# arobertlin/MinPaxos

Measured on AMD Instinct MI355X. Metric: decided+applied instances/sec (tally + KV apply + RCCL watermark all-reduce), higher is better.
Workload: dtype int32/int64

## Files before the change

minpaxos_amd/csrc/logenc.hip:

```cpp
#include <cstring>

#include "common.hpp"
#include "frames.hpp"
#include "kernels.hpp"
#include "scan.hpp"

namespace mpx {

namespace {
constexpr int kLogBlock = kFrBlock;
constexpr int kLogWindowVec = 2;
constexpr int kLogBlockBytes = kLogBlock * 16 * kLogWindowVec;
constexpr int kLogMinRec = 9;
constexpr int kLogMaxRecs = kLogBlockBytes / kLogMinRec + 2;
constexpr int kLogMaxCmds = kLogBlockBytes / 17 + 3;

__host__ __device__ __forceinline__ uint64_t zigzag(int64_t x) {
    return x < 0 ? ~((uint64_t)x << 1) : (uint64_t)x << 1;
}
__host__ __device__ __forceinline__ uint32_t hdr_bytes(int format, uint64_t ncmd) {
    return format == MPX_LOG_CATCHUP ? 8u + uvarint_len(zigzag((int64_t)ncmd)) : 12u;
}
}

struct RecBytes {
    int format;
    const uint64_t* cmd_off;
    __device__ __forceinline__ uint64_t operator()(uint64_t i) const {
        const uint64_t nc = cmd_off[i + 1] - cmd_off[i];
        return hdr_bytes(format, nc) + 17 * nc;
    }
};
struct RecOffOut {
    uint64_t* rec_off;
    uint64_t* blk_first;
    uint32_t n_blocks;
    __device__ __forceinline__ void operator()(uint64_t i, uint64_t s, uint64_t bytes) const {
        const uint64_t e = s + bytes;
        rec_off[i + 1] = e;
        for (uint64_t b = (s + kLogBlockBytes - 1) / kLogBlockBytes;
             b * kLogBlockBytes < e && b < n_blocks; ++b)
            blk_first[b] = i;
    }
};

__global__ __launch_bounds__(kLogBlock) void k_log_emit(
    int format, const mpx_log_rec* __restrict__ recs, const uint64_t* __restrict__ cmd_off,
    const uint8_t* __restrict__ op, const int64_t* __restrict__ key,
    const int64_t* __restrict__ val, uint64_t n, const uint64_t* __restrict__ rec_off,
    const uint64_t* __restrict__ blk_first, uint32_t n_blocks, uint8_t* __restrict__ out) {
    __shared__ uint64_t off[kLogMaxRecs + 1];
    __shared__ uint64_t coff[kLogMaxRecs + 1];
    __shared__ uint16_t cmap[kLogMaxCmds];
    __shared__ __attribute__((aligned(16))) uint32_t W[kLogBlockBytes / 4];
    const uint64_t total = rec_off[n];
    const uint64_t b0 = (uint64_t)blockIdx.x * kLogBlockBytes;
    if (b0 >= total) return;
    const uint64_t first = blk_first[blockIdx.x];
    const uint64_t b1 = b0 + kLogBlockBytes < total ? b0 + kLogBlockBytes : total;
    const uint64_t nr = (b1 < total && blockIdx.x + 1 < n_blocks)
                            ? blk_first[blockIdx.x + 1] - first + 1
                            : n - first;
    for (uint64_t k = threadIdx.x; k <= nr; k += kLogBlock) {
        off[k] = rec_off[first + k];
        coff[k] = cmd_off[first + k];
    }
#pragma unroll
    for (int i = 0; i < kLogWindowVec; ++i)
        reinterpret_cast<uint4*>(W)[threadIdx.x + i * kLogBlock] = make_uint4(0, 0, 0, 0);
    __syncthreads();
    uint64_t j_lo, j_hi;
    {
        const uint64_t hb0 = off[1] - off[0] - 17 * (coff[1] - coff[0]);
        const uint64_t cs0 = off[0] + hb0;
        j_lo = coff[0] + cmd_span(cs0, b0, b1).lo;
        const uint64_t L = nr - 1;
        const uint64_t hbl = off[L + 1] - off[L] - 17 * (coff[L + 1] - coff[L]);
        const uint64_t csl = off[L] + hbl;
        const uint64_t c = cmd_span(csl, b0, b1).hi;
        j_hi = coff[L] + c < coff[L + 1] ? coff[L] + c : coff[L + 1];
    }
    for (uint64_t k = threadIdx.x; k < nr; k += kLogBlock) {
        const uint64_t rs = off[k], c0 = coff[k], c1 = coff[k + 1], nc = c1 - c0;
        for (uint64_t j = c0 > j_lo ? c0 : j_lo; j < c1 && j < j_hi; ++j)
            cmap[j - j_lo] = (uint16_t)k;
        const uint32_t hb = (uint32_t)(off[k + 1] - rs - 17 * nc);
        if (rs + hb <= b0 || rs >= b1) continue;
        const mpx_log_rec m = recs[first + k];
        uint32_t h[5] = {(uint32_t)m.ballot, (uint32_t)m.status, 0u, 0u, 0u};
        if (format == MPX_LOG_DURABLE) {
            h[2] = (uint32_t)m.inst_no;
        } else {
            const uint64_t zz = zigzag((int64_t)nc);
            for (uint32_t q = 0; q + 8 < hb; ++q) h[2 + (q >> 2)] |= uvarint_byte(zz, q) << (8 * (q & 3));
        }
        image_or<kLogBlockBytes / 4>(W, (int64_t)(rs - b0), h, hb);
    }
    __syncthreads();
    for (uint64_t j = j_lo + threadIdx.x; j < j_hi; j += kLogBlock) {
        const uint32_t lo = cmap[j - j_lo];
        const uint64_t nc = coff[lo + 1] - coff[lo];
        const uint64_t cs = off[lo + 1] - 17 * nc;
        const uint64_t pos = cs + 17 * (j - coff[lo]);
        image_or_cmd<kLogBlockBytes / 4>(W, (int64_t)pos - (int64_t)b0, op[j], (uint64_t)key[j],
                                         (uint64_t)val[j]);
    }
    __syncthreads();
    window_store(W, (uint32_t)(b1 - b0), out + b0, (int)threadIdx.x);
}

uint64_t logenc_max_bytes(uint64_t n, uint64_t m) { return n * (8 + 10) + 17 * m; }

namespace {
uint64_t blocks_for(uint64_t n, uint64_t m) {
    return (logenc_max_bytes(n, m) + kLogBlockBytes - 1) / kLogBlockBytes;
}
struct LogWork {
    uint64_t* blk_first;
    uint64_t* scan_tmp;
    LogWork(Carver& c, uint64_t n, uint64_t m) {
        blk_first = c.take<uint64_t>(blocks_for(n, m));
        scan_tmp = (uint64_t*)c.take<char>(scan_scratch_bytes<uint64_t>(n ? n : 1));
    }
};
}

uint64_t logenc_work_bytes(uint64_t n, uint64_t m, Carver&& c) {
    return LogWork(c, n, m), c.bytes();
}

hipError_t launch_encode_log(int format, const mpx_log_rec* recs, uint64_t n,
                             const uint64_t* cmd_off, const uint8_t* op, const int64_t* key,
                             const int64_t* val, uint64_t m, uint8_t* out, uint64_t* rec_off,
                             void* work, uint64_t work_bytes, hipStream_t stream) {
    if (format != MPX_LOG_CATCHUP && format != MPX_LOG_DURABLE) return hipErrorInvalidValue;
    Carver c(work);
    const LogWork w(c, n, m);
    if (work_bytes < c.bytes()) return hipErrorInvalidValue;
    k_zero_u64<<<1, 1, 0, stream>>>(rec_off, 1);
    if (n == 0) return hipGetLastError();
    const uint64_t blocks = blocks_for(n, m);
    const hipError_t r = device_scan(RecBytes{format, cmd_off},
                                     RecOffOut{rec_off, w.blk_first, (uint32_t)blocks}, n,
                                     ScanSum64{}, (uint64_t)0, w.scan_tmp, stream);
    if (r != hipSuccess) return r;
    k_log_emit<<<(unsigned)blocks, kLogBlock, 0, stream>>>(format, recs, cmd_off, op, key, val, n,
                                                          rec_off, w.blk_first, (uint32_t)blocks,
                                                          out);
    return hipGetLastError();
}

}
```

Before: 23.97 billion.

## Fuse log record offset scan into emit kernel with record-tiled windows

```diff
diff --git a/minpaxos_amd/csrc/logenc.hip b/minpaxos_amd/csrc/logenc.hip
--- a/minpaxos_amd/csrc/logenc.hip
+++ b/minpaxos_amd/csrc/logenc.hip
@@ -1,7 +1,10 @@
 #include <cstring>
 
 #include "common.hpp"
+#pragma clang diagnostic push
+#pragma clang diagnostic ignored "-Wunused-function"
 #include "frames.hpp"
+#pragma clang diagnostic pop
 #include "kernels.hpp"
 #include "scan.hpp"
 
@@ -13,6 +16,7 @@
 constexpr int kLogBlockBytes = kLogBlock * 16 * kLogWindowVec;
 constexpr int kLogMinRec = 9;
 constexpr int kLogMaxRecs = kLogBlockBytes / kLogMinRec + 2;
+static_assert(kLogMaxRecs <= 65536, "cmap holds 16-bit record indices");
 constexpr int kLogMaxCmds = kLogBlockBytes / 17 + 3;
 
 __host__ __device__ __forceinline__ uint64_t zigzag(int64_t x) {
@@ -23,111 +27,202 @@
 }
 }
 
-struct RecBytes {
-    int format;
-    const uint64_t* cmd_off;
-    __device__ __forceinline__ uint64_t operator()(uint64_t i) const {
-        const uint64_t nc = cmd_off[i + 1] - cmd_off[i];
-        return hdr_bytes(format, nc) + 17 * nc;
-    }
-};
-struct RecOffOut {
-    uint64_t* rec_off;
-    uint64_t* blk_first;
-    uint32_t n_blocks;
-    __device__ __forceinline__ void operator()(uint64_t i, uint64_t s, uint64_t bytes) const {
-        const uint64_t e = s + bytes;
-        rec_off[i + 1] = e;
-        for (uint64_t b = (s + kLogBlockBytes - 1) / kLogBlockBytes;
-             b * kLogBlockBytes < e && b < n_blocks; ++b)
-            blk_first[b] = i;
-    }
-};
+constexpr int kLogTile = 512;
+constexpr int kLogPer = kLogTile / kLogBlock;
+static_assert(kLogTile % kLogBlock == 0, "a whole number of records per lane");
+constexpr int kLogScanTile = 4096;
+constexpr int kLogSub = kLogScanTile / kLogTile;
+static_assert(kLogScanTile % kLogTile == 0 && kLogSub < kLogBlock, "whole emit tiles per scan tile");
+
+__device__ __forceinline__ uint64_t uniform64(uint64_t x) {
+    return (uint64_t)__builtin_amdgcn_readfirstlane((uint32_t)(x >> 32)) << 32 |
+           __builtin_amdgcn_readfirstlane((uint32_t)x);
+}
+__device__ __forceinline__ uint64_t rec_bytes(int format, uint64_t nc) {
+    return hdr_bytes(format, nc) + 17 * nc;
+}
+
+__global__ __launch_bounds__(kLogBlock) void k_log_tile_totals(
+    int format, const uint64_t* __restrict__ cmd_off, uint64_t n, uint64_t* __restrict__ sub,
+    uint64_t* __restrict__ tot) {
+    __shared__ uint64_t ws[kLogSub][kLogBlock / kWave];
+    const int t = threadIdx.x, l = lane_id(), w = t / kWave;
+    const uint64_t r0 = (uint64_t)blockIdx.x * kLogScanTile;
+    uint64_t acc[kLogSub];
+#pragma unroll
+    for (int s = 0; s < kLogSub; ++s) {
+        acc[s] = 0;
+#pragma unroll
+        for (int j = 0; j < kLogPer; ++j) {
+            const uint64_t i = r0 + (uint64_t)(s * kLogTile + j * kLogBlock + t);
+            if (i < n) acc[s] += rec_bytes(format, cmd_off[i + 1] - cmd_off[i]);
+        }
+    }
+#pragma unroll
+    for (int s = 0; s < kLogSub; ++s) {
+#pragma unroll
+        for (int d = kWave / 2; d >= 1; d >>= 1) acc[s] += shfl_any(acc[s], l ^ d);
+        if (l == 0) ws[s][w] = acc[s];
+    }
+    __syncthreads();
+    if (t < kLogSub) {
+        uint64_t x = 0;
+        for (int v = 0; v < kLogBlock / kWave; ++v) x += ws[t][v];
+        sub[(uint64_t)blockIdx.x * kLogSub + t] = x;
+    }
+    if (t == kLogSub) {
+        uint64_t x = 0;
+        for (int s = 0; s < kLogSub; ++s)
+            for (int v = 0; v < kLogBlock / kWave; ++v) x += ws[s][v];
+        tot[blockIdx.x] = x;
+    }
+}
 
 __global__ __launch_bounds__(kLogBlock) void k_log_emit(
     int format, const mpx_log_rec* __restrict__ recs, const uint64_t* __restrict__ cmd_off,
     const uint8_t* __restrict__ op, const int64_t* __restrict__ key,
-    const int64_t* __restrict__ val, uint64_t n, const uint64_t* __restrict__ rec_off,
-    const uint64_t* __restrict__ blk_first, uint32_t n_blocks, uint8_t* __restrict__ out) {
-    __shared__ uint64_t off[kLogMaxRecs + 1];
-    __shared__ uint64_t coff[kLogMaxRecs + 1];
+    const int64_t* __restrict__ val, uint64_t n, const uint64_t* __restrict__ scan_base,
+    const uint64_t* __restrict__ sub, uint64_t* __restrict__ rec_off, uint8_t* __restrict__ out) {
+    __shared__ uint64_t off[kLogTile + 1];
+    __shared__ uint64_t coff[kLogTile + 1];
+    __shared__ uint64_t wtot[kLogBlock / kWave];
     __shared__ uint16_t cmap[kLogMaxCmds];
     __shared__ __attribute__((aligned(16))) uint32_t W[kLogBlockBytes / 4];
-    const uint64_t total = rec_off[n];
-    const uint64_t b0 = (uint64_t)blockIdx.x * kLogBlockBytes;
-    if (b0 >= total) return;
-    const uint64_t first = blk_first[blockIdx.x];
-    const uint64_t b1 = b0 + kLogBlockBytes < total ? b0 + kLogBlockBytes : total;
-    const uint64_t nr = (b1 < total && blockIdx.x + 1 < n_blocks)
-                            ? blk_first[blockIdx.x + 1] - first + 1
-                            : n - first;
-    for (uint64_t k = threadIdx.x; k <= nr; k += kLogBlock) {
-        off[k] = rec_off[first + k];
-        coff[k] = cmd_off[first + k];
-    }
-#pragma unroll
-    for (int i = 0; i < kLogWindowVec; ++i)
-        reinterpret_cast<uint4*>(W)[threadIdx.x + i * kLogBlock] = make_uint4(0, 0, 0, 0);
+    const int t = threadIdx.x, l = lane_id(), w = t / kWave;
+    const uint64_t r0 = (uint64_t)blockIdx.x * kLogTile;
+    if (r0 >= n) {
+        if (t == 0) rec_off[0] = 0;
+        return;
+    }
+    const uint32_t cnt = n - r0 < (uint64_t)kLogTile ? (uint32_t)(n - r0) : (uint32_t)kLogTile;
+    uint64_t base = scan_base[blockIdx.x / kLogSub];
+    for (uint32_t e = blockIdx.x / kLogSub * kLogSub; e < blockIdx.x; ++e) base += sub[e];
+    for (uint32_t k = t; k <= cnt; k += kLogBlock) coff[k] = cmd_off[r0 + k];
+    uint4* const W4 = reinterpret_cast<uint4*>(W);
+#pragma unroll
+    for (int i = 0; i < kLogWindowVec; ++i) W4[t + i * kLogBlock] = make_uint4(0, 0, 0, 0);
     __syncthreads();
-    uint64_t j_lo, j_hi;
     {
-        const uint64_t hb0 = off[1] - off[0] - 17 * (coff[1] - coff[0]);
-        const uint64_t cs0 = off[0] + hb0;
-        j_lo = coff[0] + cmd_span(cs0, b0, b1).lo;
-        const uint64_t L = nr - 1;
-        const uint64_t hbl = off[L + 1] - off[L] - 17 * (coff[L + 1] - coff[L]);
-        const uint64_t csl = off[L] + hbl;
-        const uint64_t c = cmd_span(csl, b0, b1).hi;
-        j_hi = coff[L] + c < coff[L + 1] ? coff[L] + c : coff[L + 1];
-    }
-    for (uint64_t k = threadIdx.x; k < nr; k += kLogBlock) {
-        const uint64_t rs = off[k], c0 = coff[k], c1 = coff[k + 1], nc = c1 - c0;
-        for (uint64_t j = c0 > j_lo ? c0 : j_lo; j < c1 && j < j_hi; ++j)
-            cmap[j - j_lo] = (uint16_t)k;
-        const uint32_t hb = (uint32_t)(off[k + 1] - rs - 17 * nc);
-        if (rs + hb <= b0 || rs >= b1) continue;
-        const mpx_log_rec m = recs[first + k];
-        uint32_t h[5] = {(uint32_t)m.ballot, (uint32_t)m.status, 0u, 0u, 0u};
-        if (format == MPX_LOG_DURABLE) {
-            h[2] = (uint32_t)m.inst_no;
-        } else {
-            const uint64_t zz = zigzag((int64_t)nc);
-            for (uint32_t q = 0; q + 8 < hb; ++q) h[2 + (q >> 2)] |= uvarint_byte(zz, q) << (8 * (q & 3));
-        }
-        image_or<kLogBlockBytes / 4>(W, (int64_t)(rs - b0), h, hb);
+        uint64_t pre[kLogPer], run = 0;
+#pragma unroll
+        for (int j = 0; j < kLogPer; ++j) {
+            const uint32_t k = (uint32_t)t * kLogPer + j;
+            pre[j] = run;
+            if (k < cnt) run += rec_bytes(format, coff[k + 1] - coff[k]);
+        }
+        const uint64_t incl = wave_incl_scan(run, ScanSum64{});
+        if (l == kWave - 1) wtot[w] = incl;
+        __syncthreads();
+        uint64_t carry = base + (incl - run);
+        for (int x = 0; x < w; ++x) carry += wtot[x];
+#pragma unroll
+        for (int j = 0; j < kLogPer; ++j) {
+            const uint32_t k = (uint32_t)t * kLogPer + j;
+            if (k < cnt) off[k] = carry + pre[j];
+        }
+        if (t == kLogBlock - 1) off[cnt] = carry + run;
     }
     __syncthreads();
-    for (uint64_t j = j_lo + threadIdx.x; j < j_hi; j += kLogBlock) {
-        const uint32_t lo = cmap[j - j_lo];
-        const uint64_t nc = coff[lo + 1] - coff[lo];
-        const uint64_t cs = off[lo + 1] - 17 * nc;
-        const uint64_t pos = cs + 17 * (j - coff[lo]);
-        image_or_cmd<kLogBlockBytes / 4>(W, (int64_t)pos - (int64_t)b0, op[j], (uint64_t)key[j],
-                                         (uint64_t)val[j]);
-    }
-    __syncthreads();
-    window_store(W, (uint32_t)(b1 - b0), out + b0, (int)threadIdx.x);
+    for (uint32_t k = t; k < cnt; k += kLogBlock) rec_off[r0 + k + 1] = off[k + 1];
+    if (r0 == 0 && t == 0) rec_off[0] = 0;
+
+    const uint64_t T0 = uniform64(off[0]), T1 = uniform64(off[cnt]);
+    const uint64_t a = (uint64_t)((uintptr_t)out & 127);
+    int64_t wb = (int64_t)((T0 + a) & ~127ull) - (int64_t)a;
+    uint32_t first = 0;
+    while (wb < (int64_t)T1) {
+        const uint64_t b0 = wb > (int64_t)T0 ? (uint64_t)wb : T0;
+        const uint64_t b1 = wb + kLogBlockBytes < (int64_t)T1 ? (uint64_t)(wb + kLogBlockBytes) : T1;
+        const uint64_t* const o = off + first;
+        const uint64_t* const co = coff + first;
+        uint32_t nr = 0;
+        for (uint32_t k = first + t;; k += kLogBlock) {
+            const int c = __syncthreads_count(k < cnt && off[k] < b1);
+            nr += (uint32_t)c;
+            if (c < kLogBlock) break;
+        }
+        nr = __builtin_amdgcn_readfirstlane(nr);
+        uint64_t j_lo;
+        uint32_t nj;
+        {
+            const uint64_t hb0 = o[1] - o[0] - 17 * (co[1] - co[0]);
+            const uint64_t cs0 = o[0] + hb0;
+            j_lo = uniform64(co[0] + cmd_span(cs0, b0, b1).lo);
+            const uint32_t L = nr - 1;
+            const uint64_t hbl = o[L + 1] - o[L] - 17 * (co[L + 1] - co[L]);
+            const uint64_t csl = o[L] + hbl;
+            const uint64_t c = cmd_span(csl, b0, b1).hi;
+            const uint64_t j_hi = co[L] + c < co[L + 1] ? co[L] + c : co[L + 1];
+            nj = __builtin_amdgcn_readfirstlane((uint32_t)(j_hi - j_lo));
+        }
+        for (uint32_t k = t; k < nr; k += kLogBlock) {
+            const uint64_t rs = o[k], c0 = co[k], c1 = co[k + 1];
+            const uint32_t nc = (uint32_t)(c1 - c0);
+            const uint32_t m0 = c0 > j_lo ? (uint32_t)(c0 - j_lo) : 0u;
+            const uint32_t m1 = c1 - j_lo < (uint64_t)nj ? (uint32_t)(c1 - j_lo) : nj;
+            for (uint32_t jj = m0; jj < m1; ++jj) cmap[jj] = (uint16_t)k;
+            const uint32_t hb = (uint32_t)(o[k + 1] - rs) - 17u * nc;
+            if (rs + hb <= b0) continue;
+            const mpx_log_rec m = recs[r0 + first + k];
+            uint32_t h[5] = {(uint32_t)m.ballot, (uint32_t)m.status, 0u, 0u, 0u};
+            if (format == MPX_LOG_DURABLE) {
+                h[2] = (uint32_t)m.inst_no;
+            } else {
+                const uint64_t zz = zigzag((int64_t)(c1 - c0));
+                for (uint32_t q = 0; q + 8 < hb; ++q) h[2 + (q >> 2)] |= uvarint_byte(zz, q) << (8 * (q & 3));
+            }
+            image_or<kLogBlockBytes / 4>(W, (int64_t)(int32_t)(uint32_t)(rs - (uint64_t)wb), h, hb);
+        }
+        __syncthreads();
+        const uint32_t* const o32 = reinterpret_cast<const uint32_t*>(o);
+        const uint32_t* const co32 = reinterpret_cast<const uint32_t*>(co);
+        const uint8_t* const wop = op + j_lo;
+        const int64_t* const wkey = key + j_lo;
+        const int64_t* const wval = val + j_lo;
+        for (uint32_t jj = t; jj < nj; jj += kLogBlock) {
+            const uint32_t lo = cmap[jj];
+            const uint32_t end = o32[2 * (lo + 1)] - (uint32_t)wb;
+            const uint32_t after = co32[2 * (lo + 1)] - ((uint32_t)j_lo + jj);
+            image_or_cmd<kLogBlockBytes / 4>(W, (int64_t)(int32_t)(end - 17u * after), wop[jj],
+                                             (uint64_t)wkey[jj], (uint64_t)wval[jj]);
+        }
+        __syncthreads();
+        const uint8_t* const S = reinterpret_cast<const uint8_t*>(W);
+        uint8_t* const wout = out + wb;
+        const uint32_t v0 = (uint32_t)(b0 - (uint64_t)wb), v1 = (uint32_t)(b1 - (uint64_t)wb);
+#pragma unroll
+        for (int i = 0; i < kLogWindowVec; ++i) {
+            const uint32_t v = (uint32_t)t + i * kLogBlock, vb = 16 * v;
+            if (vb >= v0 && vb + 16 <= v1) {
+                st_stream(reinterpret_cast<uint4*>(wout) + v, W4[v]);
+            } else if (vb + 16 > v0 && vb < v1) {
+                const uint32_t e0 = vb > v0 ? vb : v0, e1 = vb + 16 < v1 ? vb + 16 : v1;
+                for (uint32_t b = e0; b < e1; ++b) wout[b] = S[b];
+            }
+            W4[v] = make_uint4(0, 0, 0, 0);
+        }
+        first += nr - 1;
+        if (uniform64(off[first + 1]) == b1) ++first;
+        wb += kLogBlockBytes;
+    }
 }
 
 uint64_t logenc_max_bytes(uint64_t n, uint64_t m) { return n * (8 + 10) + 17 * m; }
 
 namespace {
-uint64_t blocks_for(uint64_t n, uint64_t m) {
-    return (logenc_max_bytes(n, m) + kLogBlockBytes - 1) / kLogBlockBytes;
-}
+uint64_t tiles_for(uint64_t n) { return (n + kLogTile - 1) / kLogTile; }
+uint64_t scan_tiles_for(uint64_t n) { return (n + kLogScanTile - 1) / kLogScanTile; }
 struct LogWork {
-    uint64_t* blk_first;
-    uint64_t* scan_tmp;
-    LogWork(Carver& c, uint64_t n, uint64_t m) {
-        blk_first = c.take<uint64_t>(blocks_for(n, m));
-        scan_tmp = (uint64_t*)c.take<char>(scan_scratch_bytes<uint64_t>(n ? n : 1));
+    uint64_t* scan_base;
+    uint64_t* sub;
+    LogWork(Carver& c, uint64_t n) {
+        scan_base = c.take<uint64_t>(scan_tiles_for(n) + 1);
+        sub = c.take<uint64_t>(scan_tiles_for(n) * kLogSub + 1);
     }
 };
 }
 
-uint64_t logenc_work_bytes(uint64_t n, uint64_t m, Carver&& c) {
-    return LogWork(c, n, m), c.bytes();
-}
+uint64_t logenc_work_bytes(uint64_t n, uint64_t, Carver&& c) { return LogWork(c, n), c.bytes(); }
 
 hipError_t launch_encode_log(int format, const mpx_log_rec* recs, uint64_t n,
                              const uint64_t* cmd_off, const uint8_t* op, const int64_t* key,
@@ -135,18 +230,18 @@
                              void* work, uint64_t work_bytes, hipStream_t stream) {
     if (format != MPX_LOG_CATCHUP && format != MPX_LOG_DURABLE) return hipErrorInvalidValue;
     Carver c(work);
-    const LogWork w(c, n, m);
+    const LogWork w(c, n);
     if (work_bytes < c.bytes()) return hipErrorInvalidValue;
-    k_zero_u64<<<1, 1, 0, stream>>>(rec_off, 1);
-    if (n == 0) return hipGetLastError();
-    const uint64_t blocks = blocks_for(n, m);
-    const hipError_t r = device_scan(RecBytes{format, cmd_off},
-                                     RecOffOut{rec_off, w.blk_first, (uint32_t)blocks}, n,
-                                     ScanSum64{}, (uint64_t)0, w.scan_tmp, stream);
-    if (r != hipSuccess) return r;
-    k_log_emit<<<(unsigned)blocks, kLogBlock, 0, stream>>>(format, recs, cmd_off, op, key, val, n,
-                                                          rec_off, w.blk_first, (uint32_t)blocks,
-                                                          out);
+    const uint64_t tiles = tiles_for(n), scan_tiles = scan_tiles_for(n);
+    if (tiles >= (1ull << 31)) return hipErrorInvalidValue;
+    if (n) {
+        k_log_tile_totals<<<(unsigned)scan_tiles, kLogBlock, 0, stream>>>(format, cmd_off, n, w.sub,
+                                                                         w.scan_base);
+        k_scan_totals<uint64_t, ScanSum64><<<1, kScTotT, 0, stream>>>(w.scan_base, scan_tiles,
+                                                                      ScanSum64{}, (uint64_t)0);
+    }
+    k_log_emit<<<(unsigned)(tiles ? tiles : 1), kLogBlock, 0, stream>>>(
+        format, recs, cmd_off, op, key, val, n, w.scan_base, w.sub, rec_off, out);
     return hipGetLastError();
 }
 
```

Result: no change. 23.93 billion, median of 2 (-0.1%).
